# Trippasch/CudaRayTracer

Measured on AMD Instinct MI355X. Metric: Mray/s (and ms/frame) at 1920x1080, 64 spp, depth 8, random-spheres, higher is better.
Workload: dtype f32; 1 GPU; c2: 1920x1080, 64 spp, depth 8, RTIOW final random-spheres scene; width=1920, height=1080, spp=64, depth=8, parallelism=1 GPU, kernel_variant=-1

## Files before the change

cudaraytracer_amd/_lib.py:

```python
from __future__ import annotations

import ctypes as C
import os

from . import abi

LIB_PATH = _IN_TREE = os.path.join(os.path.dirname(os.path.abspath(__file__)), "librt_hip.so")
LIB_PATH = os.environ.get("RT_HIP_LIB", LIB_PATH)

EXPORTED = [
    "LaunchKernel",
    "LaunchRandInit",
    "LaunchRenderInit",
    "rt_last_error",
    "rt_version",
    "rt_abi_version",
    "rt_set_launch_flags",
    "rt_set_device",
    "rt_scene_create",
    "rt_scene_from_reference_graph",
    "rt_scene_update_materials",
    "rt_scene_destroy",
    "rt_scene_get_info",
    "rt_render_init",
# ... 26 lines not shown
    "rt_scene_motion",
    "rt_scene_edit",
    "rt_last_kernel_ms",
    "rt_last_variant",
    "rt_last_launch_host_ms",
    "rt_set_variant",
    "rt_set_tuning",
    "rt_glibc_srand",
    "rt_glibc_rand_next",
    "rt_builtin_scene",
    "rt_camera_inputs",
    "rt_procedural_texture",
    "rt_reference_graph_flatten",
    "rt_build_host_tables",
    "rt_tile_entries_host",
]

_lib = None


class RTError(RuntimeError):
    pass


def _declare(lib: C.CDLL) -> None:
    P = C.POINTER
    vp = C.c_void_p
    lib.rt_last_error.restype = C.c_char_p
    lib.rt_version.restype = C.c_char_p
    lib.rt_set_launch_flags.argtypes = [C.c_uint32]
# ... 44 lines not shown
    lib.rt_glibc_srand.argtypes = [P(abi.GlibcRand), C.c_uint32]
    lib.rt_glibc_rand_next.argtypes = [P(abi.GlibcRand)]
    lib.rt_glibc_rand_next.restype = C.c_int32
    lib.rt_builtin_scene.argtypes = [C.c_int, C.c_uint32, P(abi.HittableDesc), P(C.c_uint32),
                                     P(abi.MaterialDesc), P(C.c_uint32)]
    lib.rt_procedural_texture.argtypes = [C.c_int, C.c_int32, C.c_int32, C.c_void_p]
    F3P = P(C.c_float)
    lib.rt_camera_inputs.argtypes = [F3P, F3P, F3P, C.c_float, C.c_float, C.c_float, F3P, F3P, P(abi.InputStruct)]
    lib.rt_reference_graph_flatten.argtypes = [vp, P(abi.HittableDesc), P(C.c_uint32), P(abi.MaterialDesc),
                                               P(C.c_uint32), P(abi.ImageDesc), P(C.c_uint32)]
    lib.rt_build_host_tables.argtypes = [P(abi.SceneDesc), P(C.c_float), P(C.c_float), P(C.c_float),
                                         P(C.c_int32), P(abi.HostTablesInfo)]
    if LIB_PATH == _IN_TREE or hasattr(lib, "rt_tile_entries_host"):
        lib.rt_tile_entries_host.argtypes = [P(abi.SceneDesc), P(abi.InputStruct), C.c_uint32, C.c_uint32, P(abi.Tiling),
                                             C.c_uint32, C.c_uint32, C.c_uint32, P(C.c_uint32)]
    lib.LaunchKernel.argtypes = [vp, C.c_uint, C.c_uint, C.c_uint, C.c_uint, vp, vp, abi.InputStruct]
    lib.LaunchKernel.restype = None
    lib.LaunchRandInit.argtypes = [vp]
    lib.LaunchRandInit.restype = None
    lib.LaunchRenderInit.argtypes = [abi.Dim3, abi.Dim3, C.c_uint, C.c_uint, vp]
    lib.LaunchRenderInit.restype = None


def lib() -> C.CDLL:
    global _lib
    if _lib is None:
        if not os.path.exists(LIB_PATH):
            raise RTError(f"{LIB_PATH} is missing: build it with `python -c 'import __graft_entry__ as g; g.build()'`")
        handle = C.CDLL(LIB_PATH)
        _declare(handle)
# ... 9 lines not shown
```

cudaraytracer_amd/abi.py:

```python
from __future__ import annotations

import ctypes as C

import numpy as np

RT_SPHERE, RT_XYRECT, RT_XZRECT, RT_YZRECT = 0, 1, 2, 3
RT_LAMBERTIAN, RT_METAL, RT_DIELECTRIC, RT_DIFFUSELIGHT = 0, 1, 2, 3
RT_CONSTANT, RT_CHECKER, RT_IMAGE = 0, 1, 2

RT_FLAG_FAITHFUL_GRID = 1 << 0
RT_FLAG_NO_STATE_WRITEBACK = 1 << 1
RT_FLAG_ACCUMULATE = 1 << 2
RT_FLAG_RIUS_LEFT_TO_RIGHT = 1 << 3
RT_FLAG_COUNT_TESTS = 1 << 4
RT_FLAG_RNG_PHILOX = 1 << 5
RT_FLAG_STATE_SOA = 1 << 6
RT_FLAG_ACCUMULATE_RESET = 1 << 7
RT_DENOISE_DEMODULATE = 1 << 0
RT_DENOISE_COLOR_IS_SUM = 1 << 1
RT_TEMPORAL_COLOR_IS_SUM = 1 << 0
RT_TEMPORAL_RESET = 1 << 1
ABI_VERSION = 14
MOTION_NO_HISTORY = (0.0, 0.0, 0.0, 0.0)
MOTION_IDENTITY = (0.0, 0.0, 0.0, 1.0)
# ... 252 lines not shown
class SceneInfo(C.Structure):
    _fields_ = [
        ("num_primitives", C.c_uint32),
        ("num_nodes", C.c_uint32),
        ("num_materials", C.c_uint32),
        ("bvh_depth", C.c_uint32),
        ("device_bytes", C.c_uint64),
    ]


class HostTablesInfo(C.Structure):
    _fields_ = [("num_nodes", C.c_uint32), ("num_prims", C.c_uint32), ("num_materials", C.c_uint32),
                ("depth", C.c_uint32)]


class GlibcRand(C.Structure):
    _fields_ = [("r", C.c_int32 * 34), ("idx", C.c_uint32)]


STATE_WORDS = 12
assert C.sizeof(CurandState) == 48
assert C.sizeof(InputStruct) == 72
assert C.sizeof(HittableDesc) == 40
assert C.sizeof(MaterialDesc) == 48
assert C.sizeof(TextureDesc) == 32


def make_inputs(origin, orientation, up, far_plane, near_plane, fov, bg_start, bg_end) -> InputStruct:
    s = InputStruct()
    s.origin[:] = [float(v) for v in origin]
# ... 13 lines not shown
```

cudaraytracer_amd/csrc/api.cpp:

```cpp
#include <hip/hip_runtime_api.h>

#include <algorithm>
#include <atomic>
#include <chrono>
#include <cmath>
#include <new>
#include <stdexcept>
#include <cstring>
#include <mutex>
#include <unordered_set>

#include "../../include/rt_reference_graph.h"
#include "rt_internal.h"
#include "rt_scene_device.h"

namespace rt {

static thread_local std::string g_last_error;

void set_error(const std::string& msg) { g_last_error = msg; }

template <class F>
static int guarded(const char* what, F&& f) {
    try {
        return f();
    } catch (const std::bad_alloc&) {
        set_error(std::string(what) + ": host allocation failed");
// ... 27 lines not shown
static void free_device(DeviceScene* s) {
    if (s->nodes) (void)hipFree((void*)s->nodes);
    if (s->nodes48) (void)hipFree((void*)s->nodes48);
    if (s->refs) (void)hipFree((void*)s->refs);
    s->nodes48 = s->refs = nullptr;
    if (s->prims) (void)hipFree((void*)s->prims);
    if (s->prims_flat) (void)hipFree((void*)s->prims_flat);
    if (s->ref_nodes) (void)hipFree((void*)s->ref_nodes);
    if (s->flat_boxes) (void)hipFree((void*)s->flat_boxes);
    if (s->flat_ref_pairs) (void)hipFree((void*)s->flat_ref_pairs);
    s->prims_flat = s->ref_nodes = s->flat_boxes = s->flat_ref_pairs = nullptr;
    if (s->bvh_ref_nodes) (void)hipFree((void*)s->bvh_ref_nodes);
    if (s->bvh_boxes) (void)hipFree((void*)s->bvh_boxes);
    if (s->bvh_ref_pairs) (void)hipFree((void*)s->bvh_ref_pairs);
    s->bvh_ref_nodes = s->bvh_boxes = s->bvh_ref_pairs = nullptr;
    if (s->prim_source) (void)hipFree((void*)s->prim_source);
    if (s->flat_source) (void)hipFree((void*)s->flat_source);
    s->prim_source = s->flat_source = nullptr;
    if (s->mats) (void)hipFree((void*)s->mats);
    if (s->imgs) (void)hipFree((void*)s->imgs);
    s->nodes = s->prims = s->mats = nullptr;
    s->imgs = nullptr;
    s->texels = nullptr;
}

int create_device_scene(const HostScene& h, rt_scene** out, std::shared_ptr<void> shared_texels) {
    rt_scene* s = new rt_scene();
    s->host = h;
    s->host.texels = std::vector<uint8_t>();
    DeviceScene& d = s->dev;
// ... 14 lines not shown
    d.prims_flat = p;
    if ((rc = upload(h.ref_nodes, &p, "hipMalloc/hipMemcpy(ref_nodes)"))) goto fail;
    d.ref_nodes = p;
    if ((rc = upload(h.flat_ref_pairs, &p, "hipMalloc/hipMemcpy(flat_ref_pairs)"))) goto fail;
    d.flat_ref_pairs = p;
    if ((rc = upload(h.flat_boxes, &p, "hipMalloc/hipMemcpy(flat_boxes)"))) goto fail;
    d.flat_boxes = p;
    if ((rc = upload(h.bvh_ref_nodes, &p, "hipMalloc/hipMemcpy(bvh_ref_nodes)"))) goto fail;
    d.bvh_ref_nodes = p;
    if ((rc = upload(h.bvh_boxes, &p, "hipMalloc/hipMemcpy(bvh_boxes)"))) goto fail;
    d.bvh_boxes = p;
    if ((rc = upload(h.bvh_ref_pairs, &p, "hipMalloc/hipMemcpy(bvh_ref_pairs)"))) goto fail;
    d.bvh_ref_pairs = p;
    d.flat_runs[0] = h.flat_runs[0];
    d.flat_runs[1] = h.flat_runs[1];
    if ((rc = upload(h.prim_source, &p, "hipMalloc/hipMemcpy(prim_source)"))) goto fail;
    d.prim_source = p;
    if ((rc = upload(h.flat_source, &p, "hipMalloc/hipMemcpy(flat_source)"))) goto fail;
    d.flat_source = p;
    if ((rc = upload(h.mats, &p, "hipMalloc/hipMemcpy(materials)"))) goto fail;
    d.mats = p;
    if ((rc = upload(h.imgs, &p, "hipMalloc/hipMemcpy(images)"))) goto fail;
    d.imgs = p;
    if (shared_texels) {
        s->texel_block = std::move(shared_texels);
    } else {
        if ((rc = upload(h.texels, &p, "hipMalloc/hipMemcpy(texels)"))) goto fail;
        if (p) s->texel_block = std::shared_ptr<void>(p, [](void* q) { (void)hipFree(q); });
    }
    d.texels = s->texel_block.get();
    d.num_nodes = h.num_nodes;
    d.num_prims = h.num_prims;
    d.num_mats = h.num_mats;
    d.num_imgs = (uint32_t)(h.imgs.size() / 4);
    d.depth = h.depth;
    d.has_image_textures = h.has_image_textures;
    d.has_textures = h.has_textures;
    d.has_rects = h.has_rects;
    d.device_bytes = (h.nodes.size() + h.nodes48.size() + h.refs.size() + h.prims.size() + h.prims_flat.size() + h.ref_nodes.size() +
                      h.flat_boxes.size() + h.flat_ref_pairs.size() + h.bvh_ref_nodes.size() + h.bvh_boxes.size() + h.bvh_ref_pairs.size() + h.mats.size() +
                      h.prim_source.size() + h.flat_source.size()) * 4 +
                     h.imgs.size() * 4 + h.texels.size();
    *out = s;
    return RT_OK;
fail:
    free_device(&d);
    delete s;
    return rc;
}

static void keep_description(rt_scene** scene, const rt_scene_desc& d, int texel_bytes) {
    static const uint8_t kHasData = 0;
    rt_scene* s = *scene;
    try {
        s->materials.assign(d.materials, d.materials + d.num_materials);
        s->images.assign(d.images, d.images + d.num_images);
// ... 326 lines not shown
int rt_build_host_tables(const rt_scene_desc* desc, float* nodes, float* prims, float* materials,
                         int32_t* prim_source, rt_host_tables_info* info) {
    if (!info) { set_error("rt_build_host_tables: info is NULL"); return RT_ERR_INVALID_ARGUMENT; }
    HostScene h;
    int rc = guarded("rt_build_host_tables", [&]() -> int {
        std::string err;
        int r = build_host_scene(desc, &h, &err);
        if (r) set_error("rt_build_host_tables: " + err);
        return r;
    });
    if (rc) return rc;
    info->num_nodes = h.num_nodes;
    info->num_prims = h.num_prims;
    info->num_materials = h.num_mats;
    info->depth = h.depth;
    if (nodes) std::copy(h.nodes.begin(), h.nodes.end(), nodes);
    if (prims) std::copy(h.prims.begin(), h.prims.begin() + (size_t)h.num_prims * 8, prims);
    if (materials) std::copy(h.mats.begin(), h.mats.end(), materials);
    if (prim_source) std::copy(h.prim_source.begin(), h.prim_source.end(), prim_source);
    return RT_OK;
}

static TemporalCamera temporal_camera(const rt_input_struct& in) {
    TemporalCamera c;
    const float* up = in.up;
    const float* fw = in.orientation;
    const float cx = up[1] * fw[2] - up[2] * fw[1];
    const float cy = -(up[0] * fw[2] - up[2] * fw[0]);
    const float cz = up[0] * fw[1] - up[1] * fw[0];
    const float inv = 1.0f / std::sqrt((cx * cx + cy * cy) + cz * cz);
    c.right[0] = inv * cx;
    c.right[1] = inv * cy;
    c.right[2] = inv * cz;
    c.fov = in.fov;
// ... 232 lines not shown
```

cudaraytracer_amd/csrc/render.hip:

```cpp
#include <hip/hip_runtime.h>

#include <cfloat>
#include <cstdio>
#include <cstdlib>
#include <cstring>
#include <atomic>
#include <map>
#include <numeric>
#include <memory>
#include <mutex>
#include <tuple>
#include <type_traits>
#include <vector>

#include "rt_epilogue.h"
#include "rt_internal.h"
#include "rt_scene_device.h"
#include "rt_tile_entry.h"

namespace rt {
namespace dev {

struct f3 {
    float x, y, z;
// ... 174 lines not shown
    const float4* bvh_ref_nodes;
    const float4* bvh_boxes;
    const float4* bvh_ref_pairs;
    uint32_t bvh_has_rects;
    uint32_t prefetch_stop;
    uint32_t group_tiles;
    uint32_t queue_base;
    uint32_t group_perm_a;
    uint32_t group_perm_b, group_perm_k;
    uint32_t queue_host_reset;
    uint32_t linger_ticks;
    uint32_t group_chunk;
    const uint4* tile_entries;
    uint32_t camera_resolve;
    uint32_t path_end_step;
};

constexpr int kStackMax = 64;
constexpr int kBlock = 256;
constexpr uint32_t kQueueCounters = 16;
constexpr uint32_t kQueueSlotWords = kQueueCounters + 3;
static_assert(kQueueCounters >= 1 && kQueueCounters <= 32, "queue heads");
constexpr uint32_t kQueueAllDone = kQueueCounters == 32 ? 0xffffffffu : (1u << kQueueCounters) - 1u;

enum StackKind { STACK_SCRATCH = 0, STACK_LDS = 1, STACK_LDS16 = 3, STACK_NONE = 4 };

struct ScratchStack {
    int s[kStackMax];
    int n;
    __device__ __forceinline__ void init(uint32_t*) { n = 0; }
// ... 1220 lines not shown
            const uint32_t rx = r[0], ry = r[1], rz = r[2], rw = r[3];
            const uint32_t e0 = rx & 0xffffu;
            if (e0 != kTileEntryRoot) {
                c.leaf = e0 == kTileEntryNone ? 0 : (int)e0;
                c.node = (int)(rx >> 16);
                const uint32_t e[6] = {ry & 0xffffu, ry >> 16, rz & 0xffffu, rz >> 16, rw & 0xffffu, rw >> 16};
                uint32_t n = 0;
#pragma unroll
                for (int i = 0; i < 6; i++)
                    if (e[i] != kTileEntryNone) {
                        stk[(kStackBase + i) * 64] = (typename RefW<WIDE>::Entry)e[i];
                        n = (uint32_t)i + 1u;
                    }
                c.sp = kStackBase + n;
            }
        }
    }
}

template <bool WIDE, class R>
__device__ __forceinline__ void v3_next_sample(const KParams& P, uint32_t x, uint32_t g, f3 contrib, R& rng,
                                               f3& col, f3& att, uint32_t& sample, uint32_t& depth, f3& ro,
                                               f3& rd, Cursor& c, uint32_t& rays, const uint32_t tile,
                                               typename RefW<WIDE>::Entry* const stk) {
    col = add_sample(rng, col, contrib);
    KParamsC* q = kparams_reload();
    const Camera cam = lane_camera(q, x, g);
    while (++sample < q->spp) {
        camera_ray(q, cam, rng, ro, rd, sample);
        att = mk(1.0f, 1.0f, 1.0f);
// ... 561 lines not shown
            bvh_replay_wave(kparams_reload(), prims, c, ro, rd, cnt, COUNT_TESTS);
        const uint64_t t_a = COUNT_TESTS ? __builtin_amdgcn_s_memtime() : 0;
        const uint32_t ntrav = COUNT_TESTS ? (uint32_t)__popcll(__ballot(c.mode == MODE_TRAV)) : 64u;
        if (c.mode == MODE_TRAV) {
            uint32_t thr = threshold;
            if (P.regen_live_frac) thr = min(thr, ((uint32_t)__popcll(__ballot(c.mode != MODE_DONE)) * P.regen_live_frac) >> 6);
            v3_traverse<COUNT_TESTS, NODES, park_words(COMPACT) * 256u, WIDE>(nrsrc, NODES == NODES_64 ? P.nodes : P.nodes48, P.refs, prims, stk, thr, ro, rd, c, cnt, ntrav, P.leaf_break);
        }
        const uint64_t t_b = COUNT_TESTS ? __builtin_amdgcn_s_memtime() : 0;
        if (COUNT_TESTS) cnt.ctrav += t_b - t_a;
        for (;;) {
            if constexpr (!WIDE && !kItemsBuild) {
                if (kparams_reload()->camera_resolve != 0u)
                    v3_resolve_camera<COUNT_TESTS, R, COMPACT>(x, g, tile, park, ro, rd, c, cnt);
            }
            if (c.mode == MODE_SHADE) {
                R rng;
                f3 col, att;
                uint32_t sample, depth, rays;
                v3_unpark<COMPACT, false>(park, rng, col, att, sample, depth, rays);
                f3 contrib;
                if (COUNT_TESTS) cnt.wshade += wave_leader();
                KParamsC* const q = kparams_reload();
                uint32_t s2[2] = {0u, 0u};
                const int res = shade<TEX, false, true>(q, prims, q->mats, q->imgs, c.hit, c.tag, c.t_best, ro, rd, att, rng,
                                                        rtl, contrib, COUNT_TESTS ? s2 : nullptr);
                if (COUNT_TESTS) {
                    cnt.s2_enter += s2[0];
                    cnt.s2_fail += s2[1];
                    if (__ballot(s2[0] != 0u) != 0) cnt.s2_pass += wave_leader();
// ... 13 lines not shown
                    park[8 * 64] += rays;
                    rays = 0u;
                    c.mode = MODE_NEED;
                } else if (ended && pend) {
                    att = contrib;
                    c.mode = MODE_ENDED;
                } else if (ended) {
                    col = mk(__uint_as_float(park[(PK_COL + 0) * 64]), __uint_as_float(park[(PK_COL + 1) * 64]),
                             __uint_as_float(park[(PK_COL + 2) * 64]));
                    v3_next_sample<WIDE>(P, x, g, contrib, rng, col, att, sample, depth, ro, rd, c, rays, tile, stk);
                    park[(PK_COL + 0) * 64] = __float_as_uint(col.x);
                    park[(PK_COL + 1) * 64] = __float_as_uint(col.y);
                    park[(PK_COL + 2) * 64] = __float_as_uint(col.z);
                } else {
                    v3_start_trace<WIDE>(P.num_nodes, c, rays);
                    if (COUNT_TESTS && P.ray_dump) dump_ray(P, depth == P.ray_dump_depth, ro, rd);
                }
                v3_park<COMPACT, false>(park, rng, col, att, sample, depth, rays);
            }
            if (!RT_REPLAY_SAME_PASS || __ballot(c.mode == MODE_REPLAY) == 0u) break;
            bvh_replay_wave(kparams_reload(), prims, c, ro, rd, cnt, COUNT_TESTS);
        }
        if constexpr (kItemsBuild) {
            const uint64_t needm = __ballot(c.mode == MODE_NEED);
            if (items && needm != 0) {
                const uint32_t item = next_item +
                    __builtin_amdgcn_mbcnt_hi((uint32_t)(needm >> 32), __builtin_amdgcn_mbcnt_lo((uint32_t)needm, 0u));
                next_item += (uint32_t)__popcll(needm);
                if (c.mode == MODE_NEED) {
                    if (item < n_items) {
                        const uint32_t p = item & 63u;
                        const uint32_t bx = tile % P.tiles_x, by = tile / P.tiles_x;
                        const uint32_t px = bx * 8u + (p & 7u), pg = global_row(P, by * 8u + (p >> 3));
                        R rng = begin_rng<R>(nullptr, 0u, pg * P.width + px);
// ... 1292 lines not shown
thread_local int g_queue_prefetch = 32;
thread_local int g_queue_guide = 0;
thread_local int g_queue_min = 16;
thread_local int g_queue_host_reset = 0;
thread_local int g_persistent_group = 2;
thread_local int g_group_tail = 0;
thread_local int g_group_order = 0;
thread_local int g_group_chunk = 1024;
thread_local int g_group_waves = 16;
thread_local int g_group_linger_us = 0;
thread_local int g_tile_entries = 1;
thread_local int g_camera_resolve = 1;
constexpr uint32_t kCameraResolveCap = 8;
constexpr int kCameraResolveMax = 32;
thread_local int g_path_end_step = 1;

struct Knob {
    int& (*at)();
    int lo, hi, step;
    bool pow2;
    const char* refusal;
};
const Knob kKnobs[] = {
    {[]() -> int& { return g_regen_threshold; }, 1, 64, 1, false, "rt_set_tuning: regen threshold must be in [1, 64]"},
    {[]() -> int& { return g_leaf_max; }, 1, kLeafMax, 1, false, "rt_set_tuning: leaf max must be in [1, 4]"},
    {[]() -> int& { return g_persistent_waves; }, 0, 16, 1, false,
     "rt_set_tuning: persistent waves per SIMD must be in [0, 16]"},
    {[]() -> int& { return g_sah_traversal_x10; }, 1, 1000, 1, false,
     "rt_set_tuning: SAH traversal cost (x10) must be in [1, 1000]"},
    {[]() -> int& { return g_lds_pad; }, 0, 65536, 4, false, "rt_set_tuning: LDS pad must be a multiple of 4 in [0, 65536]"},
// ... 644 lines not shown
    return RT_OK;
}

float rt_last_kernel_ms(void) { return g_last_ms; }

float rt_last_launch_host_ms(void) { return g_last_host_ms; }

int rt_set_variant(int variant) {
    int prev = g_variant;
    g_variant = variant;
    return prev;
}

int rt_last_variant(void) { return g_last_variant; }

int rt_set_tuning(int key, int value) {
    if (key < 0 || key >= (int)(sizeof(kKnobs) / sizeof(kKnobs[0]))) {
        set_error("rt_set_tuning: unknown key");
        return RT_ERR_INVALID_ARGUMENT;
    }
    const Knob& k = kKnobs[key];
    if (value < k.lo || value > k.hi || value % k.step || (k.pow2 && (value & (value - 1)))) {
        set_error(k.refusal);
        return RT_ERR_INVALID_ARGUMENT;
    }
    int& knob = k.at();
    const int prev = knob;
    knob = value;
    return prev;
}
// ... 228 lines not shown
        E.filled = false;
        hipLaunchKernelGGL(dev::tile_entries_kernel, dim3((P.num_tiles + 63u) / 64u), dim3(64), 0, s, (const float*)S.nodes,
                           (const float*)S.prims, F, E.rec, P.num_tiles);
        rc = hip_check(hipGetLastError(), "rt_render: tile entry kernel launch", RT_ERR_LAUNCH);
        if (rc != RT_OK) return rc;
        E.filled = true;
        E.scene_uid = S.uid;
        E.frame = F;
    }
    P.tile_entries = (const uint4*)E.rec;
    P.camera_resolve = g_camera_resolve == 1 ? kCameraResolveCap : (uint32_t)g_camera_resolve;
    P.path_end_step = (uint32_t)g_path_end_step;
    return RT_OK;
}

void fill_kernel_params(dev::KParams& P, const Variant& V, const LaunchShape& L, const DeviceScene& S) {
    P.lds_wave_words = L.wave_words;
    if (V.kernel == 5 || V.kernel == 6) fill_flat_tables(P, S);
    const int rius_trips = V.kernel == 6 ? g_rius_trips_persistent : g_rius_trips;
    P.rius_cap = rius_trips > 0 ? (uint32_t)rius_trips : 0xffffffffu;
    const uint32_t tile = V.block == 64 ? 8u : 16u;
    P.tiles_x = (P.width + tile - 1) / tile;
    P.num_tiles = P.tiles_x * ((P.local_rows + tile - 1) / tile);
}

void timing_begin(hipEvent_t ev[2], hipStream_t s) {
    if (!g_timing) return;
    (void)hipEventCreate(&ev[0]);
    (void)hipEventCreate(&ev[1]);
    (void)hipEventRecord(ev[0], s);
// ... 43 lines not shown

    hipStream_t s = (hipStream_t)stream;
    uint32_t grid = P.num_tiles;
    if (persistent) rc = setup_persistent(P, V.kernel, fn, P.num_tiles, s, L, &grid);
    if (rc != RT_OK) return rc;
    std::shared_ptr<TilePlan> plan;
    rc = bind_tile_plan(P, V.kernel, s, &plan);
    if (rc != RT_OK) return rc;
    hipEvent_t timing[2] = {nullptr, nullptr};
    timing_begin(timing, s);
    g_last_variant = variant;
    std::shared_ptr<EntryTable> entries;
    std::unique_lock<std::mutex> entries_lock;
    rc = bind_tile_entries(P, V.kernel, S, s, &entries, &entries_lock);
    if (rc != RT_OK) return rc;

    if (trial.timed) (void)hipEventRecord(trial.timed->ev[trial.slot], s);
    (void)hipGetLastError();
    hipLaunchKernelGGL(fn, dim3(grid), dim3(L.block), L.lds_bytes, s, P);
    rc = hip_check(hipGetLastError(), "rt_render: kernel launch", RT_ERR_LAUNCH);
    if (entries_lock.owns_lock()) entries_lock.unlock();
    if (rc != RT_OK && persistent)
        (void)hipMemsetAsync(P.work_counter, 0, (size_t)dev::kQueueSlotWords * P.queue_stride * 4u, s);
    if (trial.timed) (void)hipEventRecord(trial.timed->ev[trial.slot + 1], s);
    if (rc == RT_OK && plan) {
        hipLaunchKernelGGL(dev::plan_order_kernel, dim3(1), dim3(1024), 0, s, (const uint32_t*)plan->cost, plan->order,
                           P.num_tiles);
        rc = hip_check(hipGetLastError(), "rt_render: plan kernel launch", RT_ERR_LAUNCH);
        if (rc == RT_OK) plan->valid.store(true);
    }
// ... 103 lines not shown
```

cudaraytracer_amd/csrc/rt_internal.h:

```cpp
#pragma once

#include <cstdint>
#include <string>
#include <vector>

#include "../../include/rt_hip.h"

namespace rt {

constexpr int kLeafMax = 4;
constexpr uint32_t kOccupancyDepth = 12;
extern thread_local int g_leaf_max;
extern thread_local int g_sah_traversal_x10;
extern thread_local int g_texel_bytes;
constexpr int kRegStackDepth = 24;
constexpr uint32_t kFlatMaxPrims = 64;
constexpr uint32_t kRefTreeMaxDepth = 14;
constexpr uint32_t kRefTreeMaxDepthBvh = 31;

struct HostScene {
    std::vector<float> nodes;
    std::vector<float> nodes48;
    std::vector<uint32_t> refs;
    bool wide_refs = false;
// ... 6 lines not shown
    uint32_t num_mats = 0;
    uint32_t depth = 0;
    bool has_image_textures = false;
    bool has_textures = false;
    bool has_rects = false;
    std::vector<int32_t> prim_source;
    std::vector<float> prims_flat;
    std::vector<int32_t> flat_source;
    std::vector<float> ref_nodes;
    std::vector<float> flat_ref_pairs;
    std::vector<float> flat_boxes;
    uint32_t flat_runs[2] = {0u, 0u};
    std::vector<float> bvh_ref_nodes;
    std::vector<float> bvh_boxes;
    std::vector<float> bvh_ref_pairs;
};

int build_host_scene(const rt_scene_desc* desc, HostScene* out, std::string* err, bool with_texels = true);

int pack_materials(const rt_material_desc* mats, uint32_t n, uint32_t num_images, std::vector<float>* out,
                   std::string* err);

struct FlatDesc {
    std::vector<rt_hittable_desc> hittables;
    std::vector<rt_material_desc> materials;
    std::vector<rt_image_desc> images;
    rt_scene_desc desc() const {
        rt_scene_desc d;
        d.hittables = hittables.data();
        d.num_hittables = (uint32_t)hittables.size();
// ... 70 lines not shown
```

cudaraytracer_amd/csrc/rt_scene_device.h:

```cpp
#pragma once

#include <cstdint>
#include <memory>

#include "rt_internal.h"

namespace rt {

struct DeviceScene {
    const void* nodes = nullptr;
    const void* nodes48 = nullptr;
    const void* refs = nullptr;
    bool wide_refs = false;
    const void* prims = nullptr;
    const void* prims_flat = nullptr;
    const void* ref_nodes = nullptr;
    const void* flat_ref_pairs = nullptr;
    const void* flat_boxes = nullptr;
    const void* bvh_ref_nodes = nullptr;
    const void* bvh_boxes = nullptr;
    const void* bvh_ref_pairs = nullptr;
    uint32_t flat_runs[2] = {0u, 0u};
    const void* prim_source = nullptr;
    const void* flat_source = nullptr;
    const void* mats = nullptr;
    const void* imgs = nullptr;
    const void* texels = nullptr;
    uint32_t num_nodes = 0, num_prims = 0, num_mats = 0, depth = 0;
    uint32_t num_imgs = 0;
    bool has_image_textures = false;
    bool has_textures = false;
    bool has_rects = false;
    uint64_t device_bytes = 0;
    uint64_t uid = 0;
};

int create_device_scene(const HostScene& h, rt_scene** out, std::shared_ptr<void> shared_texels = nullptr);

int reference_scene_for_launch(const void* world, std::shared_ptr<rt_scene>* out, double* host_ms);
// ... 15 lines not shown
```

cudaraytracer_amd/csrc/scene_build.cpp:

```cpp
#include <algorithm>
#include <limits>
#include <functional>
#include <array>
#include <cmath>
#include <cstring>
#include <numeric>

#include "rt_internal.h"

namespace rt {
namespace {

struct Box {
    float lo[3], hi[3];
    void empty() {
        for (int i = 0; i < 3; i++) { lo[i] = INFINITY; hi[i] = -INFINITY; }
    }
    void grow(const Box& b) {
        for (int i = 0; i < 3; i++) { lo[i] = std::min(lo[i], b.lo[i]); hi[i] = std::max(hi[i], b.hi[i]); }
    }
    float area() const {
        float dx = hi[0] - lo[0], dy = hi[1] - lo[1], dz = hi[2] - lo[2];
        if (!(dx >= 0) || !(dy >= 0) || !(dz >= 0)) return 0.0f;
        return 2.0f * (dx * dy + dy * dz + dz * dx);
// ... 160 lines not shown
    }
};

void pack_prim(const rt_hittable_desc& h, float* o) {
    uint32_t tag = (uint32_t)h.type | ((uint32_t)h.material << 4);
    if (h.type == RT_SPHERE) {
        o[0] = h.center[0]; o[1] = h.center[1]; o[2] = h.center[2]; o[3] = h.radius;
        const float ar = std::fabs(h.radius);
        o[4] = h.radius * h.radius; o[5] = (ar >= 0x1p-40f && ar <= 0x1p40f) ? 1.0f / h.radius : 0.0f; o[6] = 0.0f;
    } else {
        RectGeom g = rect_geom(h);
        o[0] = g.k; o[1] = g.a0; o[2] = g.a1; o[3] = g.b0;
        o[4] = g.b1; o[5] = 0.0f; o[6] = 0.0f;
    }
    o[7] = bits_to_float(tag);
}

struct RefNode {
    float lo[3], hi[3];
    int child[2];
    uint32_t depth;
};
void ref_prim_box(const rt_hittable_desc& h, float lo[3], float hi[3]) {
    if (h.type == RT_SPHERE) {
        for (int i = 0; i < 3; i++) {
            volatile float c = h.center[i], r = h.radius;
            lo[i] = c - r;
            hi[i] = c + r;
        }
        return;
// ... 243 lines not shown
        while (((size_t)B.leaf_max << (dmin - 1)) < B.prims.size()) dmin++;
        const uint32_t target = std::max<uint32_t>(kOccupancyDepth, dmin + (dmin > kOccupancyDepth ? 1u : 0u));
        if (B.max_depth > target) {
            Builder T = B;
            T.traversal = base;
            T.depth_limit = target;
            T.build_root();
            B = std::move(T);
        }
    }
    out->num_prims = (uint32_t)B.prims.size();
    out->num_nodes = (uint32_t)B.nodes.size();
    out->depth = B.max_depth;

    out->nodes.resize((size_t)out->num_nodes * 16);
    for (uint32_t i = 0; i < out->num_nodes; i++) {
        const Builder::Node& n = B.nodes[i];
        float* o = out->nodes.data() + (size_t)i * 16;
        o[0] = n.box[0].lo[0]; o[1] = n.box[0].hi[0]; o[2] = n.box[0].lo[1]; o[3] = n.box[0].hi[1];
        o[4] = n.box[1].lo[0]; o[5] = n.box[1].hi[0]; o[6] = n.box[1].lo[1]; o[7] = n.box[1].hi[1];
        o[8] = n.box[0].lo[2]; o[9] = n.box[0].hi[2]; o[10] = n.box[1].lo[2]; o[11] = n.box[1].hi[2];
        o[12] = bits_to_float((uint32_t)n.child[0]);
        o[13] = bits_to_float((uint32_t)n.child[1]);
        o[14] = 0.0f;
        o[15] = 0.0f;
    }
    out->wide_refs = !(out->num_nodes < 0x7fffu && out->num_prims < 8192u);
    out->nodes48.resize((size_t)out->num_nodes * 12);
    out->refs.resize((size_t)out->num_nodes * (out->wide_refs ? 2 : 1));
    for (uint32_t i = 0; i < out->num_nodes; i++) {
        float* o48 = out->nodes48.data() + (size_t)i * 12;
        for (int k = 0; k < 12; k++) o48[k] = out->nodes[(size_t)i * 16 + k];
        const Builder::Node& n = B.nodes[i];
        for (int c = 0; c < 2; c++) {
            const uint32_t r = (uint32_t)n.child[c];
            float* q = o48 + 4 * c;
            q[0] = with_low_byte(q[0], r & 0xffu, false);
            q[1] = with_low_byte(q[1], (r >> 8) & 0xffu, true);
            if (out->wide_refs) {
                q[2] = with_low_byte(q[2], (r >> 16) & 0xffu, false);
                q[3] = with_low_byte(q[3], r >> 24, true);
            }
        }
        if (out->wide_refs) {
            out->refs[2 * (size_t)i] = (uint32_t)n.child[0];
            out->refs[2 * (size_t)i + 1] = (uint32_t)n.child[1];
        } else {
            out->refs[i] = ((uint32_t)n.child[0] & 0xffffu) | ((uint32_t)n.child[1] << 16);
        }
    }
    out->prims.assign((size_t)std::max(out->num_prims, 1u) * 8, 0.0f);
    out->prim_source.resize(out->num_prims);
    for (uint32_t i = 0; i < out->num_prims; i++) {
        out->prim_source[i] = B.prims[B.order[i]].src;
        pack_prim(desc->hittables[out->prim_source[i]], out->prims.data() + (size_t)i * 8);
    }
    if (out->num_prims == 0) return RT_OK;
    std::vector<int> objs;
    for (const BuildPrim& p : B.prims) objs.push_back(p.src);
    std::vector<RefNode> rn;
    build_reference_tree(desc->hittables, objs, 0, (int)objs.size(), 1, &rn);
    uint32_t rdepth = 0;
    for (const RefNode& n : rn) rdepth = std::max(rdepth, n.depth);
    if (rdepth > kRefTreeMaxDepthBvh) {
        *err = "reference BVH deeper than " + std::to_string(kRefTreeMaxDepthBvh) + " levels";
// ... 99 lines not shown
```

include/rt_hip.h:

```cpp
#ifndef RT_HIP_H
#define RT_HIP_H

#include <stddef.h>
#include <stdint.h>

#ifdef __cplusplus
extern "C" {
#endif

typedef enum rt_status {
    RT_OK = 0,
    RT_ERR_INVALID_ARGUMENT = -1,
    RT_ERR_INVALID_SCENE = -2,
    RT_ERR_OUT_OF_MEMORY = -3,
    RT_ERR_DEVICE = -4,
    RT_ERR_LAUNCH = -5,
    RT_ERR_UNSUPPORTED = -6
} rt_status;

typedef enum rt_hittable_type {
    RT_SPHERE = 0,
    RT_XYRECT = 1,
    RT_XZRECT = 2,
    RT_YZRECT = 3
// ... 356 lines not shown

int rt_reference_graph_flatten(const void* world, rt_hittable_desc* hittables, uint32_t* num_hittables,
                               rt_material_desc* materials, uint32_t* num_materials, rt_image_desc* images,
                               uint32_t* num_images);

typedef struct rt_host_tables_info {
    uint32_t num_nodes, num_prims, num_materials, depth;
} rt_host_tables_info;
int rt_build_host_tables(const rt_scene_desc* desc, float* nodes, float* prims, float* materials,
                         int32_t* prim_source, rt_host_tables_info* info);

int rt_tile_entries_host(const rt_scene_desc* desc, const rt_input_struct* inputs, uint32_t width, uint32_t height,
                         const rt_tiling* tiling, uint32_t flags, uint32_t first_tile, uint32_t num_tiles,
                         uint32_t* records);

typedef struct rt_glibc_rand { int32_t r[34]; uint32_t idx; } rt_glibc_rand;
void rt_glibc_srand(rt_glibc_rand* g, uint32_t seed);
int32_t rt_glibc_rand_next(rt_glibc_rand* g);

int rt_builtin_scene(int which, uint32_t seed, rt_hittable_desc* hittables, uint32_t* num_hittables,
                     rt_material_desc* materials, uint32_t* num_materials);

int rt_procedural_texture(int kind, int32_t width, int32_t height, uint8_t* rgb);

void rt_camera_inputs(const float position[3], const float orientation[3], const float world_up[3],
                      float fov_degrees, float near_plane, float far_plane, const float bg_start[3],
                      const float bg_end[3], rt_input_struct* out);

#ifdef __cplusplus
}
// ... 4 lines not shown
```

Before: 32270 Mray/s.

## Start secondary-ray BVH traversal from a spatial-grid leaf entry point

Builds a coarse 3D grid over the scene in which each cell maps to a BVH leaf record. The record holds that leaf plus a short chain of sibling subtrees, and extra chain nodes are appended to the node arrays so the chain covers the rest of the tree. In kernel 3 with narrow refs, every bounce ray looks up its origin's cell and seeds the traversal cursor and stack from that record instead of starting at the root. The aim is to skip the top-down descent and test nearby geometry first, which tightens tmax earlier. The cost is an extra grid and record lookup per bounce, more node data, and a risk of worse culling when the chosen leaf is far from the real hit.

After: 33670 Mray/s, median of 6. +4.3%, better.

```diff
diff --git a/cudaraytracer_amd/_lib.py b/cudaraytracer_amd/_lib.py
--- a/cudaraytracer_amd/_lib.py
+++ b/cudaraytracer_amd/_lib.py
@@ -64,6 +64,9 @@
     "rt_reference_graph_flatten",
     "rt_build_host_tables",
     "rt_tile_entries_host",
+    "rt_set_bounce_entries",
+    "rt_bounce_entries_host",
+    "rt_bounce_entry_cells",
 ]
 
 _lib = None
@@ -138,6 +141,11 @@
     if LIB_PATH == _IN_TREE or hasattr(lib, "rt_tile_entries_host"):
         lib.rt_tile_entries_host.argtypes = [P(abi.SceneDesc), P(abi.InputStruct), C.c_uint32, C.c_uint32, P(abi.Tiling),
                                              C.c_uint32, C.c_uint32, C.c_uint32, P(C.c_uint32)]
+    if LIB_PATH == _IN_TREE or hasattr(lib, "rt_set_bounce_entries"):
+        lib.rt_set_bounce_entries.argtypes = [C.c_int]
+        lib.rt_bounce_entries_host.argtypes = [P(abi.SceneDesc), P(C.c_float), P(C.c_float), P(C.c_uint32), P(C.c_uint32),
+                                               P(C.c_uint16), P(abi.BounceEntriesInfo)]
+        lib.rt_bounce_entry_cells.argtypes = [P(abi.BounceEntriesInfo), P(C.c_float), C.c_uint32, P(C.c_uint32)]
     lib.LaunchKernel.argtypes = [vp, C.c_uint, C.c_uint, C.c_uint, C.c_uint, vp, vp, abi.InputStruct]
     lib.LaunchKernel.restype = None
     lib.LaunchRandInit.argtypes = [vp]
diff --git a/cudaraytracer_amd/abi.py b/cudaraytracer_amd/abi.py
--- a/cudaraytracer_amd/abi.py
+++ b/cudaraytracer_amd/abi.py
@@ -290,6 +290,12 @@
                 ("depth", C.c_uint32)]
 
 
+class BounceEntriesInfo(C.Structure):
+    _fields_ = [("num_nodes", C.c_uint32), ("num_chain_nodes", C.c_uint32), ("num_records", C.c_uint32),
+                ("depth", C.c_uint32), ("grid_dim", C.c_uint32 * 3), ("grid_origin", C.c_float * 3),
+                ("grid_inv", C.c_float * 3), ("grid_off", C.c_float * 3)]
+
+
 class GlibcRand(C.Structure):
     _fields_ = [("r", C.c_int32 * 34), ("idx", C.c_uint32)]
 
diff --git a/cudaraytracer_amd/csrc/api.cpp b/cudaraytracer_amd/csrc/api.cpp
--- a/cudaraytracer_amd/csrc/api.cpp
+++ b/cudaraytracer_amd/csrc/api.cpp
@@ -11,6 +11,7 @@
 #include <unordered_set>
 
 #include "../../include/rt_reference_graph.h"
+#include "rt_bounce_entry.h"
 #include "rt_internal.h"
 #include "rt_scene_device.h"
 
@@ -68,6 +69,9 @@
     if (s->bvh_boxes) (void)hipFree((void*)s->bvh_boxes);
     if (s->bvh_ref_pairs) (void)hipFree((void*)s->bvh_ref_pairs);
     s->bvh_ref_nodes = s->bvh_boxes = s->bvh_ref_pairs = nullptr;
+    if (s->leaf_records) (void)hipFree((void*)s->leaf_records);
+    if (s->bounce_grid) (void)hipFree((void*)s->bounce_grid);
+    s->leaf_records = s->bounce_grid = nullptr;
     if (s->prim_source) (void)hipFree((void*)s->prim_source);
     if (s->flat_source) (void)hipFree((void*)s->flat_source);
     s->prim_source = s->flat_source = nullptr;
@@ -112,6 +116,17 @@
     d.bvh_ref_pairs = p;
     d.flat_runs[0] = h.flat_runs[0];
     d.flat_runs[1] = h.flat_runs[1];
+    if (!h.bounce_grid.empty()) {
+        if ((rc = upload(h.leaf_records, &p, "hipMalloc/hipMemcpy(leaf_records)"))) goto fail;
+        d.leaf_records = p;
+        if ((rc = upload(h.bounce_grid, &p, "hipMalloc/hipMemcpy(bounce_grid)"))) goto fail;
+        d.bounce_grid = p;
+        for (int i = 0; i < 3; i++) {
+            d.grid_dim[i] = h.grid_dim[i];
+            d.grid_inv[i] = h.grid_inv[i];
+            d.grid_off[i] = h.grid_off[i];
+        }
+    }
     if ((rc = upload(h.prim_source, &p, "hipMalloc/hipMemcpy(prim_source)"))) goto fail;
     d.prim_source = p;
     if ((rc = upload(h.flat_source, &p, "hipMalloc/hipMemcpy(flat_source)"))) goto fail;
@@ -137,7 +152,7 @@
     d.has_rects = h.has_rects;
     d.device_bytes = (h.nodes.size() + h.nodes48.size() + h.refs.size() + h.prims.size() + h.prims_flat.size() + h.ref_nodes.size() +
                       h.flat_boxes.size() + h.flat_ref_pairs.size() + h.bvh_ref_nodes.size() + h.bvh_boxes.size() + h.bvh_ref_pairs.size() + h.mats.size() +
-                      h.prim_source.size() + h.flat_source.size()) * 4 +
+                      h.prim_source.size() + h.flat_source.size() + h.leaf_records.size()) * 4 + h.bounce_grid.size() * 2 +
                      h.imgs.size() * 4 + h.texels.size();
     *out = s;
     return RT_OK;
@@ -494,10 +509,54 @@
     info->num_prims = h.num_prims;
     info->num_materials = h.num_mats;
     info->depth = h.depth;
-    if (nodes) std::copy(h.nodes.begin(), h.nodes.end(), nodes);
+    if (nodes) std::copy(h.nodes.begin(), h.nodes.begin() + (size_t)h.num_nodes * 16, nodes);
     if (prims) std::copy(h.prims.begin(), h.prims.begin() + (size_t)h.num_prims * 8, prims);
     if (materials) std::copy(h.mats.begin(), h.mats.end(), materials);
     if (prim_source) std::copy(h.prim_source.begin(), h.prim_source.end(), prim_source);
+    return RT_OK;
+}
+
+int rt_bounce_entries_host(const rt_scene_desc* desc, float* chain_nodes, float* nodes48, uint32_t* refs,
+                           uint32_t* records, uint16_t* grid, rt_bounce_entries_info* info) {
+    if (!info) { set_error("rt_bounce_entries_host: info is NULL"); return RT_ERR_INVALID_ARGUMENT; }
+    HostScene h;
+    int rc = guarded("rt_bounce_entries_host", [&]() -> int {
+        std::string err;
+        int r = build_host_scene(desc, &h, &err);
+        if (r) set_error("rt_bounce_entries_host: " + err);
+        return r;
+    });
+    if (rc) return rc;
+    std::memset(info, 0, sizeof(*info));
+    info->num_nodes = h.num_nodes;
+    info->depth = h.depth;
+    if (h.bounce_grid.empty()) return RT_OK;
+    info->num_chain_nodes = h.num_chain_nodes;
+    info->num_records = (uint32_t)(h.leaf_records.size() / 4);
+    for (int i = 0; i < 3; i++) {
+        info->grid_dim[i] = h.grid_dim[i];
+        info->grid_origin[i] = h.grid_origin[i];
+        info->grid_inv[i] = h.grid_inv[i];
+        info->grid_off[i] = h.grid_off[i];
+    }
+    if (chain_nodes) std::copy(h.chain_nodes.begin(), h.chain_nodes.end(), chain_nodes);
+    if (nodes48) std::copy(h.nodes48.begin(), h.nodes48.end(), nodes48);
+    if (refs) std::copy(h.refs.begin(), h.refs.end(), refs);
+    if (records) std::copy(h.leaf_records.begin(), h.leaf_records.end(), records);
+    if (grid) std::copy(h.bounce_grid.begin(), h.bounce_grid.end(), grid);
+    return RT_OK;
+}
+
+int rt_bounce_entry_cells(const rt_bounce_entries_info* info, const float* origins, uint32_t n, uint32_t* cells) {
+    if (!info || (n && (!origins || !cells))) { set_error("rt_bounce_entry_cells: NULL argument"); return RT_ERR_INVALID_ARGUMENT; }
+    if (info->num_records == 0 || !info->grid_dim[0] || !info->grid_dim[1] || !info->grid_dim[2]) {
+        set_error("rt_bounce_entry_cells: the scene has no bounce-entry table");
+        return RT_ERR_INVALID_ARGUMENT;
+    }
+    const float dimf[3] = {(float)(info->grid_dim[0] - 1u), (float)(info->grid_dim[1] - 1u), (float)(info->grid_dim[2] - 1u)};
+    for (uint32_t i = 0; i < n; i++)
+        cells[i] = bounce_cell(origins[3 * (size_t)i], origins[3 * (size_t)i + 1], origins[3 * (size_t)i + 2], info->grid_inv,
+                               info->grid_off, dimf, info->grid_dim);
     return RT_OK;
 }
 
diff --git a/cudaraytracer_amd/csrc/render.hip b/cudaraytracer_amd/csrc/render.hip
--- a/cudaraytracer_amd/csrc/render.hip
+++ b/cudaraytracer_amd/csrc/render.hip
@@ -212,6 +212,11 @@
     const uint4* tile_entries;
     uint32_t camera_resolve;
     uint32_t path_end_step;
+    const uint4* bounce_records;
+    const uint16_t* bounce_grid;
+    float grid_inv[3], grid_off[3];
+    float grid_max[3];
+    uint32_t grid_nx, grid_ny;
 };
 
 constexpr int kStackMax = 64;
@@ -1462,6 +1467,32 @@
                     }
                 c.sp = kStackBase + n;
             }
+        }
+    }
+}
+
+template <bool WIDE>
+__device__ __forceinline__ void v3_bounce_entry(KParamsC* q, typename RefW<WIDE>::Entry* const stk, const f3 ro, Cursor& c) {
+    if constexpr (!WIDE) {
+        const uint4* const recs = q->bounce_records;
+        if (!recs) return;
+        const float fx = fminf(fmaxf(__builtin_fmaf(ro.x, q->grid_inv[0], q->grid_off[0]), 0.0f), q->grid_max[0]);
+        const float fy = fminf(fmaxf(__builtin_fmaf(ro.y, q->grid_inv[1], q->grid_off[1]), 0.0f), q->grid_max[1]);
+        const float fz = fminf(fmaxf(__builtin_fmaf(ro.z, q->grid_inv[2], q->grid_off[2]), 0.0f), q->grid_max[2]);
+        const uint32_t cell = ((uint32_t)fz * q->grid_ny + (uint32_t)fy) * q->grid_nx + (uint32_t)fx;
+        const uint4 r = recs[q->bounce_grid[cell]];
+        const uint32_t e0 = r.x & 0xffffu;
+        if (e0 != kTileEntryRoot) {
+            c.leaf = (int)e0;
+            c.node = (int)(r.x >> 16);
+            const uint32_t e[6] = {r.y & 0xffffu, r.y >> 16, r.z & 0xffffu, r.z >> 16, r.w & 0xffffu, r.w >> 16};
+            uint32_t n = 0;
+#pragma unroll
+            for (int i = 0; i < 6; i++) n += e[i] != kTileEntryNone ? 1u : 0u;
+#pragma unroll
+            for (int i = 0; i < 6; i++)
+                if ((uint32_t)i < n) stk[(kStackBase + n - 1u - (uint32_t)i) * 64] = (typename RefW<WIDE>::Entry)e[i];
+            c.sp = kStackBase + n;
         }
     }
 }
@@ -2053,6 +2084,7 @@
                 if (kparams_reload()->camera_resolve != 0u)
                     v3_resolve_camera<COUNT_TESTS, R, COMPACT>(x, g, tile, park, ro, rd, c, cnt);
             }
+            bool bounce = false;
             if (c.mode == MODE_SHADE) {
                 R rng;
                 f3 col, att;
@@ -2096,10 +2128,12 @@
                     park[(PK_COL + 2) * 64] = __float_as_uint(col.z);
                 } else {
                     v3_start_trace<WIDE>(P.num_nodes, c, rays);
+                    bounce = true;
                     if (COUNT_TESTS && P.ray_dump) dump_ray(P, depth == P.ray_dump_depth, ro, rd);
                 }
                 v3_park<COMPACT, false>(park, rng, col, att, sample, depth, rays);
             }
+            if (bounce) v3_bounce_entry<WIDE>(kparams_reload(), stk, ro, c);
             if (!RT_REPLAY_SAME_PASS || __ballot(c.mode == MODE_REPLAY) == 0u) break;
             bvh_replay_wave(kparams_reload(), prims, c, ro, rd, cnt, COUNT_TESTS);
         }
@@ -3422,6 +3456,7 @@
 constexpr uint32_t kCameraResolveCap = 8;
 constexpr int kCameraResolveMax = 32;
 thread_local int g_path_end_step = 1;
+thread_local int g_bounce_entries = 1;
 
 struct Knob {
     int& (*at)();
@@ -4096,6 +4131,16 @@
 
 int rt_last_variant(void) { return g_last_variant; }
 
+int rt_set_bounce_entries(int on) {
+    if (on != 0 && on != 1) {
+        set_error("rt_set_bounce_entries: the value must be 0 or 1");
+        return RT_ERR_INVALID_ARGUMENT;
+    }
+    const int prev = g_bounce_entries;
+    g_bounce_entries = on;
+    return prev;
+}
+
 int rt_set_tuning(int key, int value) {
     if (key < 0 || key >= (int)(sizeof(kKnobs) / sizeof(kKnobs[0]))) {
         set_error("rt_set_tuning: unknown key");
@@ -4354,6 +4399,19 @@
     return RT_OK;
 }
 
+void bind_bounce_entries(dev::KParams& P, const int kernel, const DeviceScene& S) {
+    if (kernel != 3 || S.wide_refs || !g_bounce_entries || !S.leaf_records || !S.bounce_grid) return;
+    P.bounce_records = (const uint4*)S.leaf_records;
+    P.bounce_grid = (const uint16_t*)S.bounce_grid;
+    for (int i = 0; i < 3; i++) {
+        P.grid_inv[i] = S.grid_inv[i];
+        P.grid_off[i] = S.grid_off[i];
+        P.grid_max[i] = (float)(S.grid_dim[i] - 1u);
+    }
+    P.grid_nx = S.grid_dim[0];
+    P.grid_ny = S.grid_dim[1];
+}
+
 void fill_kernel_params(dev::KParams& P, const Variant& V, const LaunchShape& L, const DeviceScene& S) {
     P.lds_wave_words = L.wave_words;
     if (V.kernel == 5 || V.kernel == 6) fill_flat_tables(P, S);
@@ -4427,6 +4485,7 @@
     std::unique_lock<std::mutex> entries_lock;
     rc = bind_tile_entries(P, V.kernel, S, s, &entries, &entries_lock);
     if (rc != RT_OK) return rc;
+    bind_bounce_entries(P, V.kernel, S);
 
     if (trial.timed) (void)hipEventRecord(trial.timed->ev[trial.slot], s);
     (void)hipGetLastError();
diff --git a/cudaraytracer_amd/csrc/rt_bounce_entry.h b/cudaraytracer_amd/csrc/rt_bounce_entry.h
--- /dev/null
+++ b/cudaraytracer_amd/csrc/rt_bounce_entry.h
@@ -0,0 +1,21 @@
+#pragma once
+
+#include <cmath>
+#include <cstdint>
+
+#include "rt_tile_entry.h"
+
+namespace rt {
+
+constexpr uint32_t kBounceGridMaxCells = 4096;
+constexpr uint32_t kBounceChainMax = 7;
+
+RT_TILE_HD inline uint32_t bounce_cell(const float x, const float y, const float z, const float* inv, const float* off,
+                                       const float* dimf, const uint32_t* dim) {
+    const float fx = fminf(fmaxf(fmaf(x, inv[0], off[0]), 0.0f), dimf[0]);
+    const float fy = fminf(fmaxf(fmaf(y, inv[1], off[1]), 0.0f), dimf[1]);
+    const float fz = fminf(fmaxf(fmaf(z, inv[2], off[2]), 0.0f), dimf[2]);
+    return ((uint32_t)fz * dim[1] + (uint32_t)fy) * dim[0] + (uint32_t)fx;
+}
+
+}
diff --git a/cudaraytracer_amd/csrc/rt_internal.h b/cudaraytracer_amd/csrc/rt_internal.h
--- a/cudaraytracer_amd/csrc/rt_internal.h
+++ b/cudaraytracer_amd/csrc/rt_internal.h
@@ -44,6 +44,14 @@
     std::vector<float> bvh_ref_nodes;
     std::vector<float> bvh_boxes;
     std::vector<float> bvh_ref_pairs;
+    uint32_t num_chain_nodes = 0;
+    std::vector<float> chain_nodes;
+    std::vector<uint32_t> leaf_records;
+    std::vector<uint16_t> bounce_grid;
+    uint32_t grid_dim[3] = {0u, 0u, 0u};
+    float grid_origin[3] = {0.0f, 0.0f, 0.0f};
+    float grid_inv[3] = {0.0f, 0.0f, 0.0f};
+    float grid_off[3] = {0.0f, 0.0f, 0.0f};
 };
 
 int build_host_scene(const rt_scene_desc* desc, HostScene* out, std::string* err, bool with_texels = true);
diff --git a/cudaraytracer_amd/csrc/rt_scene_device.h b/cudaraytracer_amd/csrc/rt_scene_device.h
--- a/cudaraytracer_amd/csrc/rt_scene_device.h
+++ b/cudaraytracer_amd/csrc/rt_scene_device.h
@@ -23,6 +23,10 @@
     uint32_t flat_runs[2] = {0u, 0u};
     const void* prim_source = nullptr;
     const void* flat_source = nullptr;
+    const void* leaf_records = nullptr;
+    const void* bounce_grid = nullptr;
+    uint32_t grid_dim[3] = {0u, 0u, 0u};
+    float grid_inv[3] = {0.0f, 0.0f, 0.0f}, grid_off[3] = {0.0f, 0.0f, 0.0f};
     const void* mats = nullptr;
     const void* imgs = nullptr;
     const void* texels = nullptr;
diff --git a/cudaraytracer_amd/csrc/scene_build.cpp b/cudaraytracer_amd/csrc/scene_build.cpp
--- a/cudaraytracer_amd/csrc/scene_build.cpp
+++ b/cudaraytracer_amd/csrc/scene_build.cpp
@@ -6,6 +6,7 @@
 #include <cstring>
 #include <numeric>
 
+#include "rt_bounce_entry.h"
 #include "rt_internal.h"
 
 namespace rt {
@@ -198,6 +199,201 @@
         o[4] = g.b1; o[5] = 0.0f; o[6] = 0.0f;
     }
     o[7] = bits_to_float(tag);
+}
+
+void pack_node16(const Builder::Node& n, float* o) {
+    o[0] = n.box[0].lo[0]; o[1] = n.box[0].hi[0]; o[2] = n.box[0].lo[1]; o[3] = n.box[0].hi[1];
+    o[4] = n.box[1].lo[0]; o[5] = n.box[1].hi[0]; o[6] = n.box[1].lo[1]; o[7] = n.box[1].hi[1];
+    o[8] = n.box[0].lo[2]; o[9] = n.box[0].hi[2]; o[10] = n.box[1].lo[2]; o[11] = n.box[1].hi[2];
+    o[12] = bits_to_float((uint32_t)n.child[0]);
+    o[13] = bits_to_float((uint32_t)n.child[1]);
+    o[14] = 0.0f;
+    o[15] = 0.0f;
+}
+
+void pack_node48(const Builder::Node& n, const bool wide, float* o48) {
+    float o[16];
+    pack_node16(n, o);
+    for (int k = 0; k < 12; k++) o48[k] = o[k];
+    for (int c = 0; c < 2; c++) {
+        const uint32_t r = (uint32_t)n.child[c];
+        float* q = o48 + 4 * c;
+        q[0] = with_low_byte(q[0], r & 0xffu, false);
+        q[1] = with_low_byte(q[1], (r >> 8) & 0xffu, true);
+        if (wide) {
+            q[2] = with_low_byte(q[2], (r >> 16) & 0xffu, false);
+            q[3] = with_low_byte(q[3], r >> 24, true);
+        }
+    }
+}
+
+void build_bounce_entries(const Builder& B, HostScene* out) {
+    const uint32_t N = out->num_nodes;
+    if (out->wide_refs || N == 0) return;
+    struct Step { int node, side; };
+    struct Leaf { int ref; std::vector<Step> path; Box box; };
+    std::vector<Leaf> leaves;
+    std::vector<uint32_t> height(N, 0u);
+    {
+        std::vector<Step> path;
+        std::function<uint32_t(int)> walk = [&](const int n) -> uint32_t {
+            uint32_t h = 0;
+            for (int side = 0; side < 2; side++) {
+                path.push_back(Step{n, side});
+                const int c = B.nodes[n].child[side];
+                if (c < 0) leaves.push_back(Leaf{c, path, B.nodes[n].box[side]});
+                else h = std::max(h, walk(c));
+                path.pop_back();
+            }
+            return height[n] = h + 1u;
+        };
+        walk(0);
+    }
+    const auto ref_height = [&](const int r) { return r < 0 ? 0u : height[r]; };
+    std::vector<Builder::Node> chain;
+    std::vector<int> chain_of((size_t)N * 2, -1);
+    std::vector<std::array<uint32_t, kTileEntryMax>> records;
+    for (const Leaf& L : leaves) {
+        const size_t a = L.path.size();
+        std::vector<int> refs;
+        const auto sibling = [&](const size_t i) { return B.nodes[L.path[i].node].child[1 - L.path[i].side]; };
+        if (a & 1u) refs.push_back(sibling(a - 1));
+        for (size_t k = a / 2; k >= 1; k--) {
+            const Step& lo = L.path[2 * k - 1];
+            const Step& up = L.path[2 * k - 2];
+            int& id = chain_of[(size_t)lo.node * 2 + (size_t)lo.side];
+            if (id < 0) {
+                id = (int)(N + chain.size());
+                Builder::Node c;
+                c.child[0] = B.nodes[lo.node].child[1 - lo.side];
+                c.box[0] = B.nodes[lo.node].box[1 - lo.side];
+                c.child[1] = B.nodes[up.node].child[1 - up.side];
+                c.box[1] = B.nodes[up.node].box[1 - up.side];
+                chain.push_back(c);
+            }
+            refs.push_back(id);
+        }
+        std::array<uint32_t, kTileEntryMax> e;
+        e.fill(kTileEntryNone);
+        const size_t m = refs.size();
+        bool fits = m <= kBounceChainMax && m >= 1 && m - 1 <= out->depth;
+        for (size_t j = 0; j < m && fits; j++) {
+            const uint32_t h = (uint32_t)(m - 1 - j);
+            uint32_t top = 0;
+            if (refs[j] >= (int)N) {
+                const Builder::Node& c = chain[(size_t)refs[j] - N];
+                top = h + 1u + std::max(ref_height(c.child[0]), ref_height(c.child[1]));
+            } else if (refs[j] >= 0) {
+                top = h + height[refs[j]];
+            }
+            fits = top <= out->depth;
+        }
+        if (fits) {
+            e[0] = (uint32_t)L.ref & 0xffffu;
+            for (size_t j = 0; j < m; j++) e[1 + j] = (uint32_t)refs[j] & 0xffffu;
+        } else {
+            e[0] = kTileEntryRoot;
+        }
+        records.push_back(e);
+    }
+    if (N + chain.size() >= 0x7fffu || records.size() > 0xffffu) return;
+
+    Box scene;
+    scene.empty();
+    for (const BuildPrim& p : B.prims) scene.grow(p.box);
+    const auto spanning = [&](const BuildPrim& p) {
+        int wide_axes = 0;
+        for (int i = 0; i < 3; i++)
+            if (p.box.hi[i] - p.box.lo[i] > 0.5f * (scene.hi[i] - scene.lo[i])) wide_axes++;
+        return wide_axes >= 2;
+    };
+    Box g;
+    g.empty();
+    std::vector<char> candidate(leaves.size(), 0);
+    bool any = false;
+    for (size_t l = 0; l < leaves.size(); l++) {
+        const uint32_t r = ~(uint32_t)leaves[l].ref, first = r >> 2, count = (r & 3u) + 1u;
+        for (uint32_t i = first; i < first + count; i++) {
+            const BuildPrim& p = B.prims[B.order[i]];
+            if (spanning(p)) continue;
+            g.grow(p.box);
+            candidate[l] = 1;
+            any = true;
+        }
+    }
+    if (!any) {
+        g = scene;
+        std::fill(candidate.begin(), candidate.end(), 1);
+    }
+    float ext[3];
+    double volume = 1.0;
+    int flat_axes = 0;
+    for (int i = 0; i < 3; i++) {
+        ext[i] = g.hi[i] - g.lo[i];
+        if (!(ext[i] > 0.0f) || !std::isfinite(ext[i])) { ext[i] = 0.0f; flat_axes++; }
+        else volume *= (double)ext[i];
+    }
+    if (!std::isfinite(g.lo[0]) || !std::isfinite(g.lo[1]) || !std::isfinite(g.lo[2]) || !std::isfinite(volume)) return;
+    const double target = (double)std::min<size_t>(kBounceGridMaxCells, std::max<size_t>(1, 4 * leaves.size()));
+    double edge = flat_axes == 3 ? 1.0 : std::pow(volume / target, 1.0 / (double)(3 - flat_axes));
+    uint32_t dim[3];
+    for (;;) {
+        uint64_t cells = 1;
+        for (int i = 0; i < 3; i++) {
+            const double d = ext[i] > 0.0f && edge > 0.0 ? std::ceil((double)ext[i] / edge) : 1.0;
+            dim[i] = (uint32_t)std::min(std::max(d, 1.0), 256.0);
+            cells *= dim[i];
+        }
+        if (cells <= kBounceGridMaxCells) break;
+        edge *= 1.1;
+    }
+    for (int i = 0; i < 3; i++) {
+        out->grid_dim[i] = dim[i];
+        out->grid_origin[i] = g.lo[i];
+        out->grid_inv[i] = ext[i] > 0.0f ? (float)dim[i] / ext[i] : 0.0f;
+        if (!std::isfinite(out->grid_inv[i])) out->grid_inv[i] = 0.0f;
+        out->grid_off[i] = -(g.lo[i] * out->grid_inv[i]);
+    }
+    out->bounce_grid.resize((size_t)dim[0] * dim[1] * dim[2]);
+    for (uint32_t z = 0; z < dim[2]; z++)
+        for (uint32_t y = 0; y < dim[1]; y++)
+            for (uint32_t x = 0; x < dim[0]; x++) {
+                const uint32_t cell[3] = {x, y, z};
+                float c[3];
+                for (int i = 0; i < 3; i++)
+                    c[i] = out->grid_inv[i] > 0.0f ? g.lo[i] + ((float)cell[i] + 0.5f) / out->grid_inv[i] : g.lo[i];
+                size_t best = 0;
+                float best_area = INFINITY, best_dist = INFINITY;
+                for (size_t l = 0; l < leaves.size(); l++) {
+                    if (!candidate[l]) continue;
+                    const Box& b = leaves[l].box;
+                    float d2 = 0.0f;
+                    for (int i = 0; i < 3; i++) {
+                        const float d = std::max(std::max(b.lo[i] - c[i], c[i] - b.hi[i]), 0.0f);
+                        d2 += d * d;
+                    }
+                    const float area = b.area();
+                    if (d2 < best_dist || (d2 == best_dist && area < best_area)) {
+                        best = l;
+                        best_dist = d2;
+                        best_area = area;
+                    }
+                }
+                out->bounce_grid[((size_t)z * dim[1] + y) * dim[0] + x] = (uint16_t)best;
+            }
+
+    out->num_chain_nodes = (uint32_t)chain.size();
+    out->chain_nodes.resize(chain.size() * 16);
+    out->nodes48.resize((size_t)(N + chain.size()) * 12);
+    out->refs.resize((size_t)N + chain.size());
+    for (size_t i = 0; i < chain.size(); i++) {
+        pack_node16(chain[i], out->chain_nodes.data() + i * 16);
+        pack_node48(chain[i], false, out->nodes48.data() + (N + i) * 12);
+        out->refs[N + i] = ((uint32_t)chain[i].child[0] & 0xffffu) | ((uint32_t)chain[i].child[1] << 16);
+    }
+    out->leaf_records.resize(records.size() * 4);
+    for (size_t i = 0; i < records.size(); i++)
+        for (int w = 0; w < 4; w++) out->leaf_records[4 * i + w] = records[i][2 * w] | (records[i][2 * w + 1] << 16);
 }
 
 struct RefNode {
@@ -471,34 +667,13 @@
     out->depth = B.max_depth;
 
     out->nodes.resize((size_t)out->num_nodes * 16);
-    for (uint32_t i = 0; i < out->num_nodes; i++) {
-        const Builder::Node& n = B.nodes[i];
-        float* o = out->nodes.data() + (size_t)i * 16;
-        o[0] = n.box[0].lo[0]; o[1] = n.box[0].hi[0]; o[2] = n.box[0].lo[1]; o[3] = n.box[0].hi[1];
-        o[4] = n.box[1].lo[0]; o[5] = n.box[1].hi[0]; o[6] = n.box[1].lo[1]; o[7] = n.box[1].hi[1];
-        o[8] = n.box[0].lo[2]; o[9] = n.box[0].hi[2]; o[10] = n.box[1].lo[2]; o[11] = n.box[1].hi[2];
-        o[12] = bits_to_float((uint32_t)n.child[0]);
-        o[13] = bits_to_float((uint32_t)n.child[1]);
-        o[14] = 0.0f;
-        o[15] = 0.0f;
-    }
     out->wide_refs = !(out->num_nodes < 0x7fffu && out->num_prims < 8192u);
     out->nodes48.resize((size_t)out->num_nodes * 12);
     out->refs.resize((size_t)out->num_nodes * (out->wide_refs ? 2 : 1));
     for (uint32_t i = 0; i < out->num_nodes; i++) {
-        float* o48 = out->nodes48.data() + (size_t)i * 12;
-        for (int k = 0; k < 12; k++) o48[k] = out->nodes[(size_t)i * 16 + k];
+        pack_node16(B.nodes[i], out->nodes.data() + (size_t)i * 16);
+        pack_node48(B.nodes[i], out->wide_refs, out->nodes48.data() + (size_t)i * 12);
         const Builder::Node& n = B.nodes[i];
-        for (int c = 0; c < 2; c++) {
-            const uint32_t r = (uint32_t)n.child[c];
-            float* q = o48 + 4 * c;
-            q[0] = with_low_byte(q[0], r & 0xffu, false);
-            q[1] = with_low_byte(q[1], (r >> 8) & 0xffu, true);
-            if (out->wide_refs) {
-                q[2] = with_low_byte(q[2], (r >> 16) & 0xffu, false);
-                q[3] = with_low_byte(q[3], r >> 24, true);
-            }
-        }
         if (out->wide_refs) {
             out->refs[2 * (size_t)i] = (uint32_t)n.child[0];
             out->refs[2 * (size_t)i + 1] = (uint32_t)n.child[1];
@@ -506,6 +681,7 @@
             out->refs[i] = ((uint32_t)n.child[0] & 0xffffu) | ((uint32_t)n.child[1] << 16);
         }
     }
+    build_bounce_entries(B, out);
     out->prims.assign((size_t)std::max(out->num_prims, 1u) * 8, 0.0f);
     out->prim_source.resize(out->num_prims);
     for (uint32_t i = 0; i < out->num_prims; i++) {
diff --git a/include/rt_hip.h b/include/rt_hip.h
--- a/include/rt_hip.h
+++ b/include/rt_hip.h
@@ -394,6 +394,19 @@
                          const rt_tiling* tiling, uint32_t flags, uint32_t first_tile, uint32_t num_tiles,
                          uint32_t* records);
 
+int rt_set_bounce_entries(int on);
+
+typedef struct rt_bounce_entries_info {
+    uint32_t num_nodes, num_chain_nodes, num_records, depth;
+    uint32_t grid_dim[3];
+    float grid_origin[3];
+    float grid_inv[3];
+    float grid_off[3];
+} rt_bounce_entries_info;
+int rt_bounce_entries_host(const rt_scene_desc* desc, float* chain_nodes, float* nodes48, uint32_t* refs,
+                           uint32_t* records, uint16_t* grid, rt_bounce_entries_info* info);
+int rt_bounce_entry_cells(const rt_bounce_entries_info* info, const float* origins, uint32_t n, uint32_t* cells);
+
 typedef struct rt_glibc_rand { int32_t r[34]; uint32_t idx; } rt_glibc_rand;
 void rt_glibc_srand(rt_glibc_rand* g, uint32_t seed);
 int32_t rt_glibc_rand_next(rt_glibc_rand* g);
```
